# ZechengLi19/CIM

Hardware: AMD Instinct MI355X
Metric: images/sec training step (ResNet-50 VOC, ~1k proposals/img) at 1/2/4/8 GPU (higher is better)
Workload: dtype fp32

## Files before the change

### cim_amd/_lib.py

```python
import ctypes
import os

from ctypes import c_float, c_int, c_longlong, c_void_p

HERE = os.path.dirname(os.path.abspath(__file__))
LIB_PATH = os.environ.get("CIM_HIP_LIB") or os.path.join(HERE, "libcim_hip.so")

_P = c_void_p
SIGNATURES = {
    "cim_roi_align_fwd": [_P, _P, _P] + [c_int] * 6 + [c_float, c_int, c_int, _P],
    "cim_roi_align_fwd_ws": [_P, _P, _P] + [c_int] * 6 + [c_float, c_int, c_int, _P, _P],
    "cim_roi_align_maskcat_fwd_ws": [_P, _P, _P, _P] + [c_int] * 6 + [c_float, c_int, c_int, _P, _P],
    "cim_roi_align_wino7_pair_fwd": [_P, _P, _P, _P, _P] + [c_int] * 7 + [c_float, c_int, c_int, _P, _P],
    "cim_roi_align_bwd_ws": [_P, _P, _P] + [c_int] * 6 + [c_float, c_int, c_int, _P, c_int, _P, _P],
    "cim_roi_align_maskcat_bwd_ws": [_P, _P, _P, _P] + [c_int] * 6 + [c_float, c_int, c_int, _P, c_int, _P, _P],
    "cim_roi_align_bwd_workspace": [c_int, c_int, c_int, c_int],
    "cim_roi_align_bwd_scratch": [c_int, c_int, c_int, c_int, c_int],
    "cim_roi_align_bwd": [_P, _P, _P] + [c_int] * 6 + [c_float, c_int, c_int, _P, _P],
    "cim_roi_align_maskcat_fwd": [_P, _P, _P, _P] + [c_int] * 6 + [c_float, c_int, c_int, _P],
    "cim_roi_align_maskcat_bwd": [_P, _P, _P, _P] + [c_int] * 6 + [c_float, c_int, c_int, _P, _P],
    "cim_roi_align_forms": [c_int] * 9 + [_P] * 3,
    "cim_maxpool2d_out_size": [c_int, c_int, c_int, c_int],
    "cim_maxpool2d_fwd": [_P, _P, _P, c_int, c_int, c_int, c_int, c_int, c_int, _P],
    "cim_maxpool2d_bwd": [_P, _P, _P, c_int, c_int, c_int, c_int, c_int, c_int, _P],
    "cim_upsample_nearest_fwd": [_P, _P, c_int, c_int, c_int, c_int, c_int, _P],
    "cim_upsample_nearest_bwd": [_P, _P, c_int, c_int, c_int, c_int, _P],
    "cim_image_prep": [_P, c_int, c_int, _P, c_int, c_int, c_longlong, c_int, ctypes.c_double, c_int, _P, _P],
    "cim_mask_pack": [_P, _P, c_int, c_int, _P],
    "cim_mask_iou_pair": [_P, c_int, c_int, _P, _P, _P, _P],
    "cim_asy_flag": [_P, c_int, c_float, _P, _P],
    "cim_asy_prep": [_P, c_int, _P, c_int, _P, _P, _P],
    "cim_mining_step": [_P, _P, _P],
    "cim_mining_lds_bytes": [c_int, c_int],
    "cim_mining_sync_bytes": [],
    "cim_gemm_small_splits": [c_int, c_int, c_int],
    "cim_gemm_small_f32": [_P, _P, _P] + [c_int] * 8 + [_P, _P, _P, _P, _P, c_float, _P, c_int, c_int, _P, _P],
    "cim_conv1x1_bwd_workspace": [c_int, c_int, c_int, c_int],
    "cim_conv1x1_bn_act_bwd": [_P] * 8 + [c_float, c_int] + [_P] * 5 + [c_int] * 4 + [_P, _P, _P, _P, _P, c_int] + [c_int, _P, _P, c_float] + [_P] * 4 + [c_int],
    "cim_bn_part_finish": [_P, c_int, _P],
    "cim_conv3x3_nchw_splits": [c_int] * 5,
    "cim_conv3x3_nchw_f32": [_P, _P, _P] + [c_int] * 6 + [_P, _P, _P, _P, _P, c_float, _P, c_int, c_int, _P, _P],
    "cim_conv7x7_nchw_f32": [_P, _P, _P] + [c_int] * 5 + [_P, _P, _P, _P, c_float, c_int, _P],
    "cim_conv3x3_nchw_bwd_workspace": [c_int] * 6,
    "cim_conv3x3_dx_parts": [c_int] * 3,
    "cim_conv3x3_nchw_bn_act_bwd": [_P] * 8 + [c_float, c_int] + [_P] * 5 + [c_int] * 7 + [_P, _P, _P, _P, _P, c_int] + [c_int, _P, _P, c_float] + [_P] * 4,
    "cim_conv3x3_wt_multi": [_P, c_int, _P],
    "cim_bn_act_fwd": [_P, _P, _P, _P, _P, _P, c_float, _P, c_int, c_int, c_int, c_int, _P],
    "cim_bn_act_bwd_chunks": [c_int, c_int, c_int],
    "cim_bn_act_bwd": [_P, _P, _P, _P, _P, _P, c_float, _P, _P, _P, _P, c_int, c_int, c_int, c_int, _P],
    "cim_sgd_multi": [_P, _P, c_int, c_float, c_int, _P],
    "cim_adam_multi": [_P, _P, c_int, ctypes.c_double, ctypes.c_double, ctypes.c_double, c_int, _P],
    "cim_gemm_pair_splits": [c_int, c_int, c_int],
    "cim_gemm_pair": [_P, _P, _P, _P] + [c_int] * 6 + [c_int, c_int, c_int, c_int, _P, _P, _P, _P, c_int, c_int, c_int, _P],
    "cim_gemm_pair_batched": [_P, _P, _P] + [c_int] * 6 + [c_int, c_int, c_int, c_longlong, c_longlong, c_longlong,
                              _P, _P, c_int, c_int, c_int, _P],
    "cim_pair_scales": [_P, c_int, _P, _P, c_int, c_int, _P],
    "cim_pair_split": [_P, _P, c_int, c_int, c_int, c_int, c_int, c_int, c_longlong, c_longlong, _P, _P, _P],
    "cim_pair_amax": [_P, c_longlong, _P, _P],
    "cim_pair_masked_stats": [_P, _P, c_int, c_int, _P, _P, _P],
    "cim_wino7_flatten_bwd_dy_pair": [_P, _P, _P, _P, _P, _P, _P, c_int, c_int, c_int, _P],
    "cim_wino7_pair_scales": [_P, c_int, _P, c_int, _P, _P],
    "cim_wino7_input_pair": [_P, _P, _P, c_int, c_int, c_int, _P],
    "cim_wino7_filter_pair": [_P, _P, _P, c_int, c_int, _P],
    "cim_wino7_dy_pair": [_P, _P, _P, c_int, c_int, c_int, c_int, _P],
    "cim_wino7_output_amax": [_P, _P, _P, c_int, c_int, c_int, _P, _P],
    "cim_flatten_chw_pair": [_P, _P, _P, c_int, c_int, c_int, c_int, _P],
    "cim_flatten_chw_bwd_bias": [_P, _P, _P, _P, c_int, c_int, c_int, _P],
    "cim_wino_dx_adjoint_output": [_P, _P, c_int, c_int, c_int, c_int, _P],
    "cim_wino7_dx_maskfold": [_P, _P, _P, c_int, c_int, _P],
    "cim_wino_wgrad_output": [_P, _P, c_int, c_int, c_int, _P],
    "cim_losses_fwd": [_P, _P],
    "cim_linear_bias_f32": [_P, _P, _P, _P, c_int, c_int, c_int, c_int, _P, _P],
    "cim_loss_finish": [_P, c_int, _P, _P],
    "cim_loss_grad_combine": [_P] * 8 + [c_int, c_int, c_int, _P],
    "cim_head_act_fwd": [_P, _P, _P, c_int, c_int, c_int, _P],
    "cim_head_act_bwd": [_P, _P, _P, _P, c_int, c_int, c_int, _P],
    "cim_detect_ws_bytes": [c_int, c_int],
    "cim_detect_nms_limit": [_P, c_int, _P, c_int, c_int, c_float, c_float, c_int, _P, _P, _P, _P, _P],
    "cim_detect_corloc": [_P, c_int, c_int, c_int, _P, _P],
    "cim_batch_detect_ws_bytes": [_P, c_int, c_int],
    "cim_batch_detect_nms_limit": [_P, c_int, _P, _P, _P, c_int, c_int, c_float, c_float, c_int, _P, _P, _P, _P, _P, _P, _P],
    "cim_segm_words": [c_int, c_int],
    "cim_segm_pack": [_P, _P, c_longlong, c_int, c_int, c_int, _P, _P],
    "cim_segm_area": [_P, c_int, c_int, _P, _P],
    "cim_segm_rle_count": [_P, c_int, c_int, c_int, _P, _P],
    "cim_segm_rle_write": [_P, c_int, c_int, c_int, _P, _P, _P, _P],
    "cim_segm_rle_decode_ws_bytes": [c_longlong],
    "cim_segm_rle_decode": [_P, _P, _P, c_int, c_int, c_int, _P, _P, _P],
    "cim_segm_image_ws_bytes": [c_int, c_int, c_longlong],
    "cim_segm_record_bytes": [c_int, c_int, c_int, c_int],
    "cim_segm_eval_image": [_P, c_int, _P, c_int, c_int, _P, _P, c_int, c_int, c_int, c_longlong, _P, _P, _P, c_int, _P, c_int,
                            _P, _P, _P],
    "cim_segm_accumulate_ws_bytes": [c_longlong, c_int, c_int, c_int],
    "cim_segm_accumulate": [_P, c_int, c_longlong, c_int, _P, _P, _P, c_int, _P, c_int, _P, c_int, c_int, c_int, _P, _P, _P, _P,
                            _P],
    "cim_poly_ws_bytes": [c_int, c_int, c_int],
    "cim_poly_fill": [_P, _P, _P, _P, c_int, c_int, c_longlong, c_int, c_int, c_int, _P, _P, _P],
    "cim_box_image_ws_bytes": [c_int, c_int, c_longlong],
    "cim_box_eval_image": [_P, c_int, _P, c_int, _P, _P, c_int, c_int, c_int, c_longlong, _P, _P, _P, c_int, _P, c_int, _P, _P, _P],
    "cim_voc_match": [_P, _P, c_int, _P, _P, c_int, _P, c_int, ctypes.c_double, c_int, _P, _P, _P, _P, _P],
    "cim_voc_ap_ws_bytes": [c_longlong],
    "cim_voc_ap": [_P, _P, _P, c_longlong, _P, _P, c_int, _P, c_int, _P, _P, c_int, _P, _P, _P, _P, _P, _P],
    "cim_prop_ws_bytes": [c_int, c_int, c_int],
    "cim_prop_prepare": [_P, c_int, c_int, c_int, c_int, _P, _P, _P, _P, _P, _P, _P],
    "cim_prop_assign": [_P, _P, c_int, c_int, c_int, _P, _P, _P, c_int, c_int, _P, _P, _P],
}

ABI_VERSION = 16
_lib = None


class CimHipError(RuntimeError):
    pass


def load():
    global _lib
    if _lib is not None:
        return _lib
    import torch
    if not os.path.exists(LIB_PATH):
        raise CimHipError(
            "libcim_hip.so not found at %s - build it with `python -m cim_amd.build` "
            "(there is no CPU fallback for the CIM hot path)" % LIB_PATH)
    lib = ctypes.CDLL(LIB_PATH)
    lib.cim_last_error.restype = ctypes.c_char_p
    lib.cim_last_error.argtypes = []
    lib.cim_abi_version.restype = c_int
    if lib.cim_abi_version() != ABI_VERSION:
        raise CimHipError("%s exports ABI %d, this package binds ABI %d: rebuild with `python -m cim_amd.build`"
                          % (LIB_PATH, lib.cim_abi_version(), ABI_VERSION))
    for name, argtypes in SIGNATURES.items():
        fn = getattr(lib, name)
        fn.argtypes = argtypes
        fn.restype = c_longlong if name in ("cim_conv1x1_bwd_workspace", "cim_conv3x3_nchw_bwd_workspace", "cim_roi_align_bwd_workspace", "cim_roi_align_bwd_scratch", "cim_mining_lds_bytes", "cim_mining_sync_bytes", "cim_detect_ws_bytes") or name in _LONG_RETURNING else c_int
    _lib = lib
    return lib


_LONG_RETURNING = {"cim_segm_rle_decode_ws_bytes", "cim_segm_image_ws_bytes", "cim_segm_record_bytes", "cim_segm_accumulate_ws_bytes", "cim_prop_ws_bytes", "cim_poly_ws_bytes", "cim_box_image_ws_bytes",
                   "cim_voc_ap_ws_bytes", "cim_batch_detect_ws_bytes"}
VALUE_RETURNING = _LONG_RETURNING | {"cim_segm_words"} | {"cim_maxpool2d_out_size", "cim_conv3x3_dx_parts", "cim_mining_sync_bytes", "cim_conv1x1_bwd_workspace", "cim_conv3x3_nchw_bwd_workspace", "cim_conv3x3_nchw_splits", "cim_gemm_small_splits", "cim_mining_lds_bytes", "cim_bn_act_bwd_chunks", "cim_gemm_pair_splits", "cim_roi_align_bwd_workspace", "cim_roi_align_bwd_scratch", "cim_detect_ws_bytes"}


PURE = {"cim_maxpool2d_out_size", "cim_conv3x3_dx_parts", "cim_gemm_small_splits", "cim_conv3x3_nchw_splits", "cim_conv1x1_bwd_workspace", "cim_conv3x3_nchw_bwd_workspace",
        "cim_bn_act_bwd_chunks", "cim_gemm_pair_splits"}
_PURE_VALUES = {}


def call(name, *args):
    if name in PURE:
        key = (name,) + args
        v = _PURE_VALUES.get(key)
# ... 22 lines not shown
```

### cim_amd/csrc/winograd.hip

```cpp
#include "common.h"
#include "../../include/cim_hip.h"
#include "wino7_tile.h"

namespace {

__device__ __forceinline__ float4 f4(float v) { return make_float4(v, v, v, v); }
__device__ __forceinline__ void fma2(float2& a, float s, float2 v) { a.x = fmaf(s, v.x, a.x); a.y = fmaf(s, v.y, a.y); }

typedef float w7_v2 __attribute__((ext_vector_type(2)));
typedef float w7_v4 __attribute__((ext_vector_type(4)));

constexpr int W7_VOUT = 4;
constexpr int W7_VDX = 2;
constexpr int W7_VMF = 1;
constexpr int W7_MF_WAVES = 1;
constexpr int W7_FB_WAVES = 3;
constexpr int W7_WG_CI = 4;

template <int N> struct w7_vec;
template <> struct w7_vec<1> { typedef float T; };
template <> struct w7_vec<2> { typedef float2 T; };
template <> struct w7_vec<4> { typedef float4 T; };
__device__ __forceinline__ void w7_store(float* p, float v) { __builtin_nontemporal_store(v, p); }
__device__ __forceinline__ void w7_store(float* p, float2 v) { __builtin_nontemporal_store(w7_v2{v.x, v.y}, reinterpret_cast<w7_v2*>(p)); }
// ... 286 lines not shown
__device__ __forceinline__ void w7_dx_tile(const float* __restrict__ M, size_t MC, size_t rc, VT (&acc)[7][7]) {
    constexpr int NA = W7::NP[KA], NB = W7::NP[KB], P = 7, Q0 = W7::QOFF[KA * 2 + KB];
    VT q[NA][NB];
#pragma unroll
    for (int i = 0; i < NA; ++i)
#pragma unroll
        for (int j = 0; j < NB; ++j) q[i][j] = vload_once<VT>(M + (size_t)(Q0 + i * NB + j) * MC + rc);
#pragma unroll
    for (int k = 0; k < NA; ++k) {
        const int yy = W7::IN0[KA] + k;
        if (yy < 0 || yy >= P) continue;
        VT t[NB];
#pragma unroll
        for (int j = 0; j < NB; ++j) {
            vzero(t[j]);
#pragma unroll
            for (int i = 0; i < NA; ++i)
                if (W7_BT[KA][i][k] != 0.0f) vfma(t[j], W7_BT[KA][i][k], q[i][j]);
        }
#pragma unroll
        for (int l = 0; l < NB; ++l) {
            const int xx = W7::IN0[KB] + l;
            if (xx < 0 || xx >= P) continue;
#pragma unroll
            for (int j = 0; j < NB; ++j)
                if (W7_BT[KB][j][l] != 0.0f) vfma(acc[yy][xx], W7_BT[KB][j][l], t[j]);
        }
    }
}

__global__ __launch_bounds__(256) void wino7_dx_kernel(const float* __restrict__ M, float* __restrict__ dx, int R, int C) {
    constexpr int VW = W7_VDX;
    typedef typename w7_vec<VW>::T VT;
    const int r = blockIdx.x;
    const size_t MC = (size_t)R * C;
    for (int c = (blockIdx.y * 256 + threadIdx.x) * VW; c < C; c += gridDim.y * 256 * VW) {
        VT acc[7][7];
#pragma unroll
        for (int y = 0; y < 7; ++y)
#pragma unroll
            for (int x = 0; x < 7; ++x) vzero(acc[y][x]);
        const size_t rc = (size_t)r * C + c;
        w7_for_all_tiles([&](auto t) __attribute__((always_inline)) { w7_dx_tile<t.KA, t.KB, VT>(M, MC, rc, acc); });
#pragma unroll
        for (int y = 0; y < 7; ++y)
#pragma unroll
            for (int x = 0; x < 7; ++x) w7_store(dx + (((size_t)r * 7 + y) * 7 + x) * C + c, acc[y][x]);
    }
}

__global__ __launch_bounds__(256, W7_MF_WAVES) void wino7_dx_maskfold_kernel(const float* __restrict__ M, const float* __restrict__ masks,
                                                                float* __restrict__ dbox, int R, int Cb) {
    constexpr int VW = W7_VMF;
    typedef typename w7_vec<VW>::T VT;
    const int r = blockIdx.x;
    const size_t C2 = 2 * (size_t)Cb, MC = (size_t)R * C2;
    const float* __restrict__ mk = masks + (size_t)r * 49;
    for (int c = (blockIdx.y * 256 + threadIdx.x) * VW; c < Cb; c += gridDim.y * 256 * VW) {
        VT acc[7][7];
#pragma unroll
        for (int y = 0; y < 7; ++y)
#pragma unroll
            for (int x = 0; x < 7; ++x) vzero(acc[y][x]);
        const size_t rc = (size_t)r * C2 + c;
        w7_for_all_tiles([&](auto t) __attribute__((always_inline)) { w7_dx_tile<t.KA, t.KB, VT>(M, MC, rc + Cb, acc); });
#pragma unroll
        for (int y = 0; y < 7; ++y)
#pragma unroll
            for (int x = 0; x < 7; ++x) {
                const float m = mk[y * 7 + x];
                VT z;
                vzero(z);
                vfma(z, m, acc[y][x]);
                acc[y][x] = z;
            }
        w7_for_all_tiles([&](auto t) __attribute__((always_inline)) { w7_dx_tile<t.KA, t.KB, VT>(M, MC, rc, acc); });
#pragma unroll
        for (int y = 0; y < 7; ++y)
#pragma unroll
            for (int x = 0; x < 7; ++x) w7_store(dbox + (((size_t)r * 7 + y) * 7 + x) * Cb + c, acc[y][x]);
    }
}

template <int KA, int KB, typename VT>
__device__ __forceinline__ void w7_wgrad_tile(const float* __restrict__ dU, size_t KN, size_t idx, VT (&acc)[3][3]) {
    constexpr int NA = W7::NP[KA], NB = W7::NP[KB], Q0 = W7::QOFF[KA * 2 + KB];
    VT s[3][NB];
#pragma unroll
    for (int a = 0; a < 3; ++a)
#pragma unroll
        for (int j = 0; j < NB; ++j) vzero(s[a][j]);
#pragma unroll
    for (int i = 0; i < NA; ++i)
#pragma unroll
        for (int j = 0; j < NB; ++j) {
            const VT q = vload_once<VT>(dU + (size_t)(Q0 + i * NB + j) * KN + idx);
#pragma unroll
            for (int a = 0; a < 3; ++a)
                if (W7_AW[KA][a][i] != 0.0f) vfma(s[a][j], W7_AW[KA][a][i], q);
        }
#pragma unroll
    for (int a = 0; a < 3; ++a)
#pragma unroll
        for (int b = 0; b < 3; ++b)
#pragma unroll
            for (int j = 0; j < NB; ++j)
                if (W7_AW[KB][b][j] != 0.0f) vfma(acc[a][b], W7_AW[KB][b][j], s[a][j]);
}

__global__ __launch_bounds__(256) void wino7_wgrad_out_kernel(const float* __restrict__ dU, float* __restrict__ dW, int Cout,
                                                              int Cin) {
    const size_t idx = (size_t)blockIdx.x * 256 + threadIdx.x;
    const size_t KN = (size_t)Cin * Cout;
    if (idx >= KN) return;
    const int ci = (int)(idx / Cout), co = (int)(idx % Cout);
    float acc[3][3];
#pragma unroll
    for (int a = 0; a < 3; ++a)
#pragma unroll
        for (int b = 0; b < 3; ++b) acc[a][b] = 0.0f;
    w7_for_all_tiles([&](auto t) __attribute__((always_inline)) { w7_wgrad_tile<t.KA, t.KB, float>(dU, KN, idx, acc); });
    float* dst = dW + ((size_t)co * Cin + ci) * 9;
#pragma unroll
    for (int a = 0; a < 3; ++a)
#pragma unroll
        for (int b = 0; b < 3; ++b) dst[a * 3 + b] = acc[a][b];
}

__global__ __launch_bounds__(64 * W7_WG_CI) void wino7_wgrad_out_rows_kernel(const float* __restrict__ dU, float* __restrict__ dW,
                                                                                 int Cout, int Cin) {
    constexpr int NCI = W7_WG_CI, ROW = 9 * NCI;
    __shared__ float t[64][ROW + 1];
    const int lane = threadIdx.x & 63, w = threadIdx.x >> 6;
    const int co0 = blockIdx.x * 64, ci0 = blockIdx.y * NCI;
    const size_t KN = (size_t)Cin * Cout;
    const size_t idx = (size_t)(ci0 + w) * Cout + co0 + lane;
    float acc[3][3];
#pragma unroll
    for (int a = 0; a < 3; ++a)
#pragma unroll
        for (int b = 0; b < 3; ++b) acc[a][b] = 0.0f;
    w7_for_all_tiles([&](auto t) __attribute__((always_inline)) { w7_wgrad_tile<t.KA, t.KB, float>(dU, KN, idx, acc); });
#pragma unroll
    for (int a = 0; a < 3; ++a)
#pragma unroll
        for (int b = 0; b < 3; ++b) t[lane][w * 9 + a * 3 + b] = acc[a][b];
    __syncthreads();
    for (int e = threadIdx.x; e < 64 * ROW; e += 64 * NCI) {
        const int row = e / ROW, col = e - row * ROW;
        dW[((size_t)(co0 + row) * Cin + ci0) * 9 + col] = t[row][col];
    }
}

__global__ __launch_bounds__(256) void flatten_chw_bwd_kernel(const float* __restrict__ src, const float* __restrict__ y,
                                                              float* __restrict__ dst, int PP, int C, float* __restrict__ bsum) {
    __shared__ float t[64][65];
    const int r = blockIdx.x, c0 = blockIdx.y * 64, tid = threadIdx.x;
    const size_t base = (size_t)r * PP * C;
    for (int e = tid; e < PP * 64; e += 256) {
        const int c = e / PP, p = e - c * PP;
        t[p][c] = src[base + (size_t)c0 * PP + e];
    }
    __syncthreads();
    float part = 0.0f;
    for (int e = tid; e < PP * 64; e += 256) {
        const int p = e >> 6, c = e & 63;
        const size_t o = base + (size_t)p * C + c0 + c;
        const float v = (y == nullptr || y[o] > 0.0f) ? t[p][c] : 0.0f;
        dst[o] = v;
        part += v;
    }
    if (bsum != nullptr) {
        __syncthreads();
        t[tid >> 6][tid & 63] = part;
        __syncthreads();
        if (tid < 64) bsum[(size_t)r * C + c0 + tid] = (t[0][tid] + t[1][tid]) + (t[2][tid] + t[3][tid]);
    }
}

__global__ __launch_bounds__(256) void flatten_chw_pair_kernel(const float* __restrict__ src, float* __restrict__ dst, int R,
                                                               int PP, int C, const float* __restrict__ scale) {
    __shared__ float t[64][65];
    const int r = blockIdx.x, c0 = blockIdx.y * 64, tid = threadIdx.x;
    float* out = dst + (size_t)r * PP * C + (size_t)c0 * PP;
    const int chunks = PP * 8;
    if (r >= R) {
        for (int q = tid; q < chunks * 2; q += 256) *reinterpret_cast<float4*>(out + q * 4) = make_float4(0.f, 0.f, 0.f, 0.f);
        return;
    }
    const size_t base = (size_t)r * PP * C;
    for (int e = tid; e < PP * 64; e += 256) {
        const int p = e >> 6, c = e & 63;
        t[p][c] = src[base + (size_t)p * C + c0 + c];
    }
    __syncthreads();
    const float s = scale[0];
    for (int q = tid; q < chunks; q += 256) {
        float v[8];
#pragma unroll
        for (int k = 0; k < 8; ++k) {
            const int e = q * 8 + k, c = e / PP, p = e - c * PP;
            v[k] = t[p][c] * s;
        }
        unsigned hh[4], ll[4];
#pragma unroll
        for (int e = 0; e < 4; ++e) cim::pair_split2(v[2 * e], v[2 * e + 1], hh[e], ll[e]);
        const w7_u4 h = {hh[0], hh[1], hh[2], hh[3]}, l = {ll[0], ll[1], ll[2], ll[3]};
        *reinterpret_cast<w7_u4*>(out + q * 8) = h;
        *reinterpret_cast<w7_u4*>(out + q * 8 + 4) = l;
    }
}

}

extern "C" int cim_wino_wgrad_output(const float* dU, float* dW, int Cout, int Cin, int tile, void* stream) {
    CIM_CHECK_ARG(dU && dW && Cout > 0 && Cin > 0);
    CIM_CHECK_ARG(tile == 7);
    const size_t n = (size_t)Cout * Cin;
    if (Cout % 64 == 0 && Cin % W7_WG_CI == 0 && Cin / W7_WG_CI <= 65535)
        hipLaunchKernelGGL(wino7_wgrad_out_rows_kernel, dim3(Cout / 64, Cin / W7_WG_CI), dim3(64 * W7_WG_CI), 0, cim::as_stream(stream), dU,
                           dW, Cout, Cin);
    else hipLaunchKernelGGL(wino7_wgrad_out_kernel, dim3((unsigned)((n + 255) / 256)), dim3(256), 0, cim::as_stream(stream), dU, dW, Cout, Cin);
    CIM_CHECK_LAUNCH();
    return 0;
}

extern "C" int cim_wino_dx_adjoint_output(const float* M, float* dx, int R, int P, int C, int tile, void* stream) {
    CIM_CHECK_ARG(R > 0 && P > 0 && P <= 64 && C > 0 && C % 4 == 0);
    CIM_CHECK_ARG(M && dx && tile == 7 && P == 7 && R <= 2147483647);
    int chunks = (C + 256 * W7_VDX - 1) / (256 * W7_VDX);
    if (chunks > 4) chunks = 4;
    hipLaunchKernelGGL(wino7_dx_kernel, dim3(R, chunks), dim3(256), 0, cim::as_stream(stream), M, dx, R, C);
    CIM_CHECK_LAUNCH();
    return 0;
}

extern "C" int cim_wino7_dx_maskfold(const float* M, const float* masks, float* dbox, int R, int Cb, void* stream) {
    CIM_CHECK_ARG(M && masks && dbox && R > 0 && Cb > 0 && Cb % 4 == 0);
    int chunks = (Cb + 256 * W7_VMF - 1) / (256 * W7_VMF);
    if (chunks > 4) chunks = 4;
    hipLaunchKernelGGL(wino7_dx_maskfold_kernel, dim3(R, chunks), dim3(256), 0, cim::as_stream(stream), M, masks, dbox, R, Cb);
    CIM_CHECK_LAUNCH();
    return 0;
}

extern "C" int cim_wino7_pair_scales(const uint32_t* amax, int n_amax, const uint32_t* amax_mul, int kind, float* scale, void* stream) {
    CIM_CHECK_ARG(amax && scale && kind >= 0 && kind <= 3 && n_amax >= 1 && n_amax <= 65536);
    hipLaunchKernelGGL(wino7_pair_scales_kernel, dim3(1), dim3(128), 0, cim::as_stream(stream), amax, n_amax, amax_mul, kind, scale);
    CIM_CHECK_LAUNCH();
    return 0;
}

extern "C" int cim_wino7_input_pair(const float* x, void* V, const float* scale, int R, int Rs, int C, void* stream) {
    CIM_CHECK_ARG(x && V && scale && R > 0 && Rs >= R && C > 0 && C % 8 == 0);
    hipLaunchKernelGGL(wino7_input_pair_kernel, dim3(Rs, 4), dim3(256), 0, cim::as_stream(stream), x, (float*)V, R, Rs, C, scale);
    CIM_CHECK_LAUNCH();
    return 0;
}

extern "C" int cim_wino7_filter_pair(const float* W, void* U, const float* scale, int Cout, int Cin, void* stream) {
    CIM_CHECK_ARG(W && U && scale && Cout > 0 && Cin > 0 && Cin % 8 == 0);
    const size_t n = (size_t)Cout * Cin;
    hipLaunchKernelGGL(wino7_filter_pair_kernel, dim3((unsigned)((n + 255) / 256)), dim3(256), 0, cim::as_stream(stream), W,
                       (float*)U, Cout, Cin, scale);
    CIM_CHECK_LAUNCH();
    return 0;
}

extern "C" int cim_wino7_dy_pair(const float* dy, void* D, const float* scale, int R, int Rs, int C, int adjoint, void* stream) {
    CIM_CHECK_ARG(dy && D && scale && R > 0 && Rs >= R && C > 0 && C % 8 == 0);
    if (adjoint) hipLaunchKernelGGL(wino7_dy_pair_kernel<true>, dim3(Rs, 4), dim3(256), 0, cim::as_stream(stream), dy, (float*)D, R, Rs, C, scale);
    else hipLaunchKernelGGL(wino7_dy_pair_kernel<false>, dim3(Rs, 4), dim3(256), 0, cim::as_stream(stream), dy, (float*)D, R, Rs, C, scale);
    CIM_CHECK_LAUNCH();
    return 0;
}

extern "C" int cim_wino7_flatten_bwd_dy_pair(const float* dX, const float* relu_y, void* E, const float* scale_e, void* D,
                                             const float* scale_d, float* bias_partial, int R, int Rs, int C, void* stream) {
    CIM_CHECK_ARG(dX && (E || D) && (!E || scale_e) && (!D || scale_d) && R > 0 && Rs >= R && C > 0 && C % 256 == 0 && C / 256 <= 65535);
    hipLaunchKernelGGL(wino7_flatten_bwd_dy_pair_kernel, dim3(Rs, C / 256), dim3(256), 0, cim::as_stream(stream), dX, relu_y, (float*)E,
                       (float*)D, bias_partial, R, Rs, C, scale_e, scale_d);
    CIM_CHECK_LAUNCH();
    return 0;
}

extern "C" int cim_wino7_output_amax(const float* M, const float* bias, float* y, int R, int C, int relu, uint32_t* y_amax,
                                     void* stream) {
    CIM_CHECK_ARG(M && y && R > 0 && C > 0 && C % 4 == 0);
    hipLaunchKernelGGL(wino7_output_kernel, dim3(R, 4), dim3(256), 0, cim::as_stream(stream), M, bias, y, R, C, relu, y_amax);
    CIM_CHECK_LAUNCH();
    return 0;
}

extern "C" int cim_flatten_chw_pair(const float* src, void* dst, const float* scale, int R, int Rs, int PP, int C, void* stream) {
    CIM_CHECK_ARG(src && dst && scale && R > 0 && Rs >= R && PP > 0 && PP <= 64 && C > 0 && C % 64 == 0 && C / 64 <= 65535);
    hipLaunchKernelGGL(flatten_chw_pair_kernel, dim3(Rs, C / 64), dim3(256), 0, cim::as_stream(stream), src, (float*)dst, R, PP, C, scale);
    CIM_CHECK_LAUNCH();
    return 0;
}

extern "C" int cim_flatten_chw_bwd_bias(const float* src, const float* relu_y, float* dst, float* bias_partial, int R, int PP,
                                        int C, void* stream) {
    CIM_CHECK_ARG(src && dst && R > 0 && PP > 0 && PP <= 64 && C > 0 && C % 64 == 0 && C / 64 <= 65535);
    hipLaunchKernelGGL(flatten_chw_bwd_kernel, dim3(R, C / 64), dim3(256), 0, cim::as_stream(stream), src, relu_y, dst, PP, C, bias_partial);
    CIM_CHECK_LAUNCH();
    return 0;
}
// ... 1 lines not shown
```

### cim_amd/ops/maskfuse_pair.py

```python
import torch
from torch.autograd import Function

from .. import _lib
from . import chain
from . import gemm as G
from . import pair

NPOS = 121
DEFER_DW = True
DW_WGS = 256
DW_FORM = 1
DW_FORM1_WGS = 0
import collections as _collections
SCHEDULE = _collections.Counter()


def supported(cat, wc, w1, w2):
    r, cin, p, q = cat.shape
    cout = wc.shape[0]
    return (cat.is_cuda and p == 7 and q == 7 and cin % 32 == 0 and cout % 64 == 0 and wc.shape[1] == cin
            and w1.shape[1] == cout * 49 and w1.shape[0] % 32 == 0 and w2.shape[1] == w1.shape[0] and w2.shape[0] % 32 == 0)


def _weight_amax(w, rows, cols):
# ... 170 lines not shown
            G.run_postponed(gcat.device)
        return dfeat, None, None, dwc, dbc, dw1, db1, dw2, db2, None, None, None


def _head_backward(ctx, dY2, ofs, fold_masks=None):
    if True:
        (y, Y1, Y2, Vb, Vs, Ub, Us, W1b, W1s, W2b, W2s, Xb, Xs, Y1b, Y1s) = ctx.saved_tensors
        r, cin, cout, h1, h2, p = ctx.dims
        dev, rp = y.device, pair.pad32(r)
        V = pair.Pair(Vb, r, cin, NPOS, Vs)
        Up = pair.Pair(Ub, cout, cin, NPOS, Us)
        W1p, W2p = pair.Pair(W1b, h1, cout * p * p, 1, W1s), pair.Pair(W2b, h2, h1, 1, W2s)
        Xp, Y1p = pair.Pair(Xb, r, cout * p * p, 1, Xs), pair.Pair(Y1b, r, h1, 1, Y1s)
        need_x, need_wc, need_w1, need_w2 = ctx.needs_input_grad[0], ctx.needs_input_grad[1 + ofs], ctx.needs_input_grad[3 + ofs], ctx.needs_input_grad[5 + ofs]
        cur, side = torch.cuda.current_stream(dev), G._side_stream(dev)
        overlap = G.OVERLAP and not torch.cuda.is_current_stream_capturing()

        def on_side(fn):
            if not overlap:
                return fn()
            side.wait_stream(cur)
            with torch.cuda.stream(side):
                out = fn()
            return out

        def publish(w, dw):
            pub = publisher
            if pub is None or dw is None or not isinstance(w, torch.nn.Parameter) or not w.is_leaf:
                return dw
            if pub(w, dw, side if overlap else cur):
                published.append(dw)
                SCHEDULE["weight_gradients_published_early"] += 1
                return None
            return dw

        published = []
        publisher = G.publisher_for(ctx.weights[1])
        if publisher is not None and chain.restricted_pass(ctx, (1 + ofs, 3 + ofs, 5 + ofs)):
            publisher = None
        late = []
        restricted = chain.restricted_pass(ctx, (1 + ofs, 3 + ofs, 5 + ofs))
        defer = DEFER_DW and G.DEFER_DW and not restricted
        run_late = overlap and defer and DW_WGS > 0

        def side_grad(slot, w, fn):
            if run_late:
                late.append((slot, w, fn))
                return None
            return publish(w, on_side(fn))

        wc_p, w1_p, w2_p = ctx.weights
        dcat = dwc = dbc = dw1 = db1 = dw2 = db2 = None
        needed = [w for w, need in ((w2_p, need_w2), (w1_p, need_w1), (wc_p, need_wc)) if need]
        will_postpone = (run_late and G.POSTPONE_DW and publisher is None and len(needed) > 0
                         and all(isinstance(w, torch.nn.Parameter) for w in needed))
        bc_p, b1_p, b2_p = getattr(ctx, "biases", (None, None, None))
        late_bias = []

        def bias_sum(b_p, part):
            if part is None:
                return None
            if will_postpone and isinstance(b_p, torch.nn.Parameter):
                late_bias.append((b_p, part, torch.empty(part.shape[1], dtype=part.dtype, device=part.device)))
                return None
            return part.sum(dim=0)
        dy_keep = []
        am = torch.zeros(3, dtype=torch.int32, device=dev)
        dY2 = dY2.contiguous()
        db2 = bias_sum(b2_p, pair.masked_stats(dY2, Y2, am[0:1], ctx.has_bias[2] and ctx.needs_input_grad[6 + ofs], reduce=False))
        dY2p = pair.split(dY2, r, h2, h2, scale=pair.scales_from(am[0:1], 1), relu_y=Y2)
        if need_w2:
            dw2 = side_grad(2, w2_p, lambda limit=0, form=0: pair.gemm(dY2p, Y1p, h2, h1, rp, True, False, limit=limit, form=form))
        dY1 = pair.gemm(dY2p, W2p, r, h1, h2, False, False)
        db1 = bias_sum(b1_p, pair.masked_stats(dY1, Y1, am[1:2], ctx.has_bias[1] and ctx.needs_input_grad[4 + ofs], reduce=False))
        dY1p = pair.split(dY1, r, h1, h1, scale=pair.scales_from(am[1:2], 1), relu_y=Y1)
        if need_w1:
            dw1 = side_grad(1, w1_p, lambda limit=0, form=0: pair.gemm(dY1p, Xp, h1, cout * p * p, rp, True, False, limit=limit, form=form))
        if need_x or need_wc or (ctx.has_bias[0] and ctx.needs_input_grad[2 + ofs]):
            dX = pair.gemm(dY1p, W1p, r, cout * p * p, h1, False, False, c_amax=am[2:3], balance=True)
            st = _lib.stream_ptr()
            want_dbc = ctx.has_bias[0] and ctx.needs_input_grad[2 + ofs]
            bpart = torch.empty((r, cout), dtype=torch.float32, device=dev) if want_dbc else None
            fused = FUSE_DY and cout % 256 == 0 and p == 7
            E = D = dy = None
            if fused:
                if need_x:
                    sE = torch.empty(NPOS, dtype=torch.float32, device=dev)
                    _lib.call("cim_wino7_pair_scales", am[2:3].data_ptr(), 1, None, 3, sE.data_ptr(), st)
                    E = pair.Pair(torch.empty((NPOS, rp, cout), dtype=torch.int32, device=dev), r, cout, NPOS, sE)
                if need_wc:
                    sD = torch.empty(NPOS, dtype=torch.float32, device=dev)
                    _lib.call("cim_wino7_pair_scales", am[2:3].data_ptr(), 1, None, 2, sD.data_ptr(), st)
                    D = pair.Pair(torch.empty((NPOS, rp, cout), dtype=torch.int32, device=dev), r, cout, NPOS, sD)
                if E is not None or D is not None:
                    _lib.call("cim_wino7_flatten_bwd_dy_pair", dX.data_ptr(), y.data_ptr(), _lib.ptr(E.buf if E is not None else None),
                              _lib.ptr(E.scale if E is not None else None), _lib.ptr(D.buf if D is not None else None),
                              _lib.ptr(D.scale if D is not None else None),
                              _lib.ptr(bpart), r, rp, cout, st)
                else:
                    fused = False
            if not fused:
                dy = torch.empty((r, p, p, cout), dtype=torch.float32, device=dev)
                _lib.call("cim_flatten_chw_bwd_bias", dX.data_ptr(), y.data_ptr(), dy.data_ptr(), _lib.ptr(bpart), r, p * p, cout, st)
            del dX
            if want_dbc:
                dbc = bias_sum(bc_p, bpart)
            if need_wc:
                def wgrad(limit=0, form=0, D=D):
                    st2 = _lib.stream_ptr()
                    if D is None:
                        sD = torch.empty(NPOS, dtype=torch.float32, device=dev)
                        _lib.call("cim_wino7_pair_scales", am[2:3].data_ptr(), 1, None, 2, sD.data_ptr(), st2)
                        D = pair.Pair(torch.empty((NPOS, rp, cout), dtype=torch.int32, device=dev), r, cout, NPOS, sD)
                        _lib.call("cim_wino7_dy_pair", dy.data_ptr(), D.buf.data_ptr(), sD.data_ptr(), r, rp, cout, 0, st2)
                    dU = pair.gemm(V, D, cin, cout, rp, True, False, limit=limit, form=form)
                    dw = torch.empty((cout, cin, 3, 3), dtype=torch.float32, device=dev)
                    _lib.call("cim_wino_wgrad_output", dU.data_ptr(), dw.data_ptr(), cout, cin, 7, st2)
                    return dw
                dwc = side_grad(0, wc_p, wgrad)
            if need_x:
                if E is None:
                    sE = torch.empty(NPOS, dtype=torch.float32, device=dev)
                    _lib.call("cim_wino7_pair_scales", am[2:3].data_ptr(), 1, None, 3, sE.data_ptr(), st)
                    E = pair.Pair(torch.empty((NPOS, rp, cout), dtype=torch.int32, device=dev), r, cout, NPOS, sE)
                    _lib.call("cim_wino7_dy_pair", dy.data_ptr(), E.buf.data_ptr(), sE.data_ptr(), r, rp, cout, 1, st)
                M2 = pair.gemm(E, Up, r, cin, cout, False, False, balance=True)
                if fold_masks is None:
                    dxp = torch.empty((r, p, p, cin), dtype=torch.float32, device=dev)
                    _lib.call("cim_wino_dx_adjoint_output", M2.data_ptr(), dxp.data_ptr(), r, p, cin, 7, st)
                else:
                    dxp = torch.empty((r, p, p, cin // 2), dtype=torch.float32, device=dev)
                    _lib.call("cim_wino7_dx_maskfold", M2.data_ptr(), fold_masks.data_ptr(), dxp.data_ptr(), r, cin // 2, st)
                dcat = dxp.permute(0, 3, 1, 2)
            dy_keep = [t for t in ((dy,) if D is None else (D.buf, D.scale)) if t is not None]
            if overlap:
                for t in dy_keep:
                    t.record_stream(side)
        keep_alive = [t for t in (V.buf, V.scale, Xp.buf, Xp.scale, Y1p.buf, Y1p.scale, dY2p.buf, dY2p.scale, dY1p.buf, dY1p.scale, am)
                      if t is not None] + dy_keep
        if late:
            late.sort(key=lambda e: -e[1].numel())

            def launch(defer):
                c2 = torch.cuda.current_stream(dev)
                late_st = G._late_stream(dev) if publisher is None else side
                late_st.wait_stream(c2)
                if late_st is not side:
                    late_st.wait_stream(side)
                    for t in keep_alive:
                        t.record_stream(late_st)
                with torch.cuda.stream(late_st):
                    limit = (G.LATE_CUS or DW_WGS) if publisher is None else 0
                    form = DW_FORM
                    if form == 1:
                        limit = DW_FORM1_WGS
                    SCHEDULE["late_launches_chunked" if publisher is None else "late_launches_whole_products"] += 1
                    got = {slot: publish(w, fn(limit, form)) for slot, w, fn in late}
                    if defer:
                        for b_p, part, out in late_bias:
                            part.record_stream(late_st)
                            out.record_stream(late_st)
                            torch.sum(part, dim=0, out=out)
                if defer:
                    for b_p, part, out in late_bias:
                        G.defer_side_join(dev, b_p, out, part)
                    keep = [t for t in (V.buf, V.scale, Xp.buf, Xp.scale, Y1p.buf, Y1p.scale, dY2p.buf, dY2p.scale, dY1p.buf,
                                        dY1p.scale, am) if t is not None] + dy_keep
                    for slot, w, _ in late:
                        if got[slot] is not None:
                            G.defer_side_join(dev, w, got[slot], *keep)
                return got

            if G.POSTPONE_DW and publisher is None and all(isinstance(w, torch.nn.Parameter) for _, w, _ in late):
                SCHEDULE["late_launches_postponed_behind_roi_align"] += 1
                G.postpone(dev, lambda: launch(True))
            else:
                assert not late_bias, "bias partial sums were left to a postponed launch that does not happen"
                got = launch(False)
                dwc, dw1, dw2 = got.get(0, dwc), got.get(1, dw1), got.get(2, dw2)
        else:
            assert not late_bias, "bias partial sums were left to a postponed launch that does not happen"
        if overlap:
            for t in [V.buf, V.scale, Xp.buf, Xp.scale, Y1p.buf, Y1p.scale, dY2p.buf, dY2p.scale, dY1p.buf, dY1p.scale, am] + dy_keep:
                if t is not None:
                    t.record_stream(side)
            if defer:
                keep = [V.buf, Xp.buf, Y1p.buf, dY2p.buf, dY1p.buf] + dy_keep
                for w, t in ((w2_p, dw2), (w1_p, dw1), (wc_p, dwc)):
                    if t is not None and isinstance(w, torch.nn.Parameter):
                        G.defer_side_join(dev, w, t, *[k for k in keep if k is not None])
                dw2 = None if isinstance(w2_p, torch.nn.Parameter) else dw2
                dw1 = None if isinstance(w1_p, torch.nn.Parameter) else dw1
                dwc = None if isinstance(wc_p, torch.nn.Parameter) else dwc
                if any(t is not None for t in (dw2, dw1, dwc)):
                    cur.wait_stream(side)
            else:
                cur.wait_stream(side)
                for t in (dw2, dw1, dwc):
                    if t is not None:
                        t.record_stream(cur)
        return dcat, dwc, dbc, dw1, db1, dw2, db2


def maskfuse_head(cat, conv, fc1, fc2, feat_amax):
    return MaskFusePairFunction.apply(cat, conv.weight, conv.bias, fc1.weight, fc1.bias, fc2.weight, fc2.bias, feat_amax)


def roi_supported(x, conv_w, fc1_w, fc2_w, resolution):
    c, h, w = x.shape[1], x.shape[2], x.shape[3]
    cout = conv_w.shape[0]
    return (x.is_cuda and x.dtype == torch.float32 and resolution == 7 and c % 32 == 0 and h <= 128 and w <= 128 and h * w * c < (1 << 30)
            and cout % 64 == 0 and conv_w.shape[1] == 2 * c and fc1_w.shape[1] == cout * 49 and fc1_w.shape[0] % 32 == 0
            and fc2_w.shape[1] == fc1_w.shape[0] and fc2_w.shape[0] % 32 == 0)


def maskfuse_roi_head(x, rois, masks, conv, fc1, fc2, feat_amax, spatial_scale, sampling_ratio):
    return MaskFuseRoiPairFunction.apply(x, rois, masks, conv.weight, conv.bias, fc1.weight, fc1.bias, fc2.weight, fc2.bias,
# ... 2 lines not shown
```

### include/cim_hip.h

```cpp
#ifndef CIM_HIP_H
#define CIM_HIP_H

#include <stdint.h>

#ifdef __cplusplus
extern "C" {
#endif

const char* cim_last_error(void);
int cim_abi_version(void);

int cim_roi_align_fwd(const float* feat, const float* rois, float* out,
                      int B, int C, int H, int W, int K, int P,
                      float spatial_scale, int sampling_ratio, int aligned, void* stream);

long long cim_roi_align_bwd_workspace(int K, int P, int H, int W);
int cim_roi_align_bwd(const float* grad_out, const float* rois, float* grad_in,
                      int B, int C, int H, int W, int K, int P,
                      float spatial_scale, int sampling_ratio, int aligned, float* workspace, void* stream);

int cim_roi_align_fwd_ws(const float* feat, const float* rois, float* out,
                         int B, int C, int H, int W, int K, int P,
                         float spatial_scale, int sampling_ratio, int aligned, float* workspace, void* stream);
int cim_roi_align_maskcat_fwd_ws(const float* feat, const float* rois, const float* masks, float* cat,
// ... 139 lines not shown
int cim_prop_prepare(const uint8_t* masks_u8, int N, int H, int W, int S, uint64_t* packed, int32_t* boxes, int32_t* area,
                     uint8_t* small, int32_t* empty_flag, void* ws, void* stream);
int cim_prop_assign(const uint64_t* packed, const int32_t* area, int N, int H, int W, const int32_t* rows, const int32_t* cols,
                    const int32_t* classes, int P, int C, float* mat, void* ws, void* stream);

int cim_image_prep(const uint8_t* src_bgr, int h, int w, float* dst, int H, int W, long long plane_stride, int row_stride,
                   double inv_scale, int hflip, const float* mean_std6_host, void* stream);

int cim_maxpool2d_out_size(int in, int k, int stride, int pad);
int cim_maxpool2d_fwd(const float* x, float* y, int* idx, int NC, int H, int W, int k, int stride, int pad, void* stream);
int cim_maxpool2d_bwd(const float* dy, const int* idx, float* dx, int NC, int H, int W, int k, int stride, int pad, void* stream);
int cim_upsample_nearest_fwd(const float* x, float* y, int NC, int H, int W, int scale, int accumulate, void* stream);
int cim_upsample_nearest_bwd(const float* dy, float* dx, int NC, int H, int W, int scale, void* stream);

int cim_gemm_small_splits(int M, int N, int K);
int cim_gemm_small_f32(const float* A, const float* B, float* C, int M, int N, int K, int lda, int ldb, int ldc,
                       int a_mcontig, int b_kcontig, float* x_raw, const float* gamma, const float* beta,
                       const float* mean, const float* var, float eps, const float* residual, int relu, int splits,
                       float* workspace, void* stream);

long long cim_conv1x1_bwd_workspace(int B, int cin, int cout, int hw);
int cim_conv1x1_bn_act_bwd(const float* dy, const float* y, const float* x_raw, const float* x, const float* w,
                           const float* gamma, const float* mean, const float* var, float eps, int relu,
                           float* dres, float* dgamma, float* dbeta, float* dx, float* dw, int B, int cin, int cout, int hw,
                           float* workspace, void* stream, void* side_stream, void* fork_event, void* join_event, int join,
                           int dy_is_dconv, const float* in_gamma, const float* in_var, float in_eps,
                           const float* in_xr, const float* in_mean, float* in_part, const float* dx_add, int dx_add_w);
typedef struct { const float* part; const float* var; float eps; float* dgamma; float* dbeta; int images; int parts; int channels; } cim_bn_part_desc;
int cim_bn_part_finish(const cim_bn_part_desc* descs, int n, void* stream);

int cim_conv3x3_nchw_splits(int cin, int cout, int H, int W, int stride);
int cim_conv3x3_nchw_f32(const float* x, const float* w, float* y, int cin, int cout, int H, int W, int stride, int dilation,
                         float* x_raw, const float* gamma, const float* beta, const float* mean, const float* var, float eps,
                         const float* residual, int relu, int splits, float* workspace, void* stream);
int cim_conv7x7_nchw_f32(const float* x, const float* w, float* y, int cin, int cout, int H, int W, int stride,
                         const float* gamma, const float* beta, const float* mean, const float* var, float eps, int relu,
                         void* stream);
long long cim_conv3x3_nchw_bwd_workspace(int B, int cin, int cout, int H, int W, int stride);
int cim_conv3x3_dx_parts(int H, int W, int stride);
int cim_conv3x3_nchw_bn_act_bwd(const float* dy, const float* y, const float* x_raw, const float* x, const float* w,
                                const float* gamma, const float* mean, const float* var, float eps, int relu, float* dres,
                                float* dgamma, float* dbeta, float* dx, float* dw, int B, int cin, int cout, int H, int W,
                                int stride, int dilation, float* workspace, void* stream, void* side_stream, void* fork_event,
                                void* join_event, int join, int dy_is_dconv, const float* in_gamma, const float* in_var, float in_eps,
                                const float* in_xr, const float* in_mean, float* in_part, const float* wt_ready);
typedef struct { const float* w; float* wt; int cin; int cout; } cim_wt_desc;
int cim_conv3x3_wt_multi(const cim_wt_desc* descs, int n, void* stream);

int cim_bn_act_fwd(const float* x, const float* res, const float* gamma, const float* beta, const float* mean,
                   const float* var, float eps, float* y, int N, int C, int HW, int relu, void* stream);
int cim_bn_act_bwd_chunks(int N, int C, int HW);
int cim_bn_act_bwd(const float* dy, const float* y, const float* x, const float* gamma, const float* mean,
                   const float* var, float eps, float* dx, float* dres, float* dgamma, float* dbeta,
                   int N, int C, int HW, int relu, void* stream);

int cim_gemm_pair_splits(int M, int N, int K);
int cim_gemm_pair(const void* A, const void* B, float* C, const float* bias, int M, int N, int K,
                  int lda, int ldb, int ldc, int a_mcontig, int b_kcontig, int relu, int splits, float* workspace,
                  const float* a_scale, const float* b_scale, uint32_t* c_amax, int max_workgroups, int products, int form,
                  void* stream);
int cim_gemm_pair_batched(const void* A, const void* B, float* C, int M, int N, int K,
                          int lda, int ldb, int ldc, int a_mcontig, int b_kcontig,
                          int batch, long long a_bs, long long b_bs, long long c_bs,
                          const float* a_scale, const float* b_scale, int max_workgroups, int products, int form, void* stream);
int cim_pair_scales(const uint32_t* amax, int n_amax, const float* factor, float* scale, int n, int reduce_all, void* stream);
int cim_pair_split(const float* X, void* P, int rows, int rows_pad, int cols, int ld, int ldp, int batch,
                   long long x_bs, long long p_bs, const float* scale, const float* relu_y, void* stream);
int cim_pair_amax(const float* X, long long n, uint32_t* amax, void* stream);
int cim_pair_masked_stats(const float* dy, const float* y, int rows, int cols, float* part, uint32_t* amax, void* stream);

int cim_wino7_pair_scales(const uint32_t* amax, int n_amax, const uint32_t* amax_mul, int kind, float* scale, void* stream);
int cim_wino7_input_pair(const float* x, void* V, const float* scale, int R, int Rs, int C, void* stream);
int cim_wino7_filter_pair(const float* W, void* U, const float* scale, int Cout, int Cin, void* stream);
int cim_wino7_dy_pair(const float* dy, void* D, const float* scale, int R, int Rs, int C, int adjoint, void* stream);
int cim_wino7_flatten_bwd_dy_pair(const float* dX, const float* relu_y, void* E, const float* scale_e, void* D, const float* scale_d,
                                  float* bias_partial, int R, int Rs, int C, void* stream);
int cim_wino7_output_amax(const float* M, const float* bias, float* y, int R, int C, int relu, uint32_t* y_amax, void* stream);
int cim_flatten_chw_pair(const float* src, void* dst, const float* scale, int R, int Rs, int PP, int C, void* stream);
int cim_flatten_chw_bwd_bias(const float* src, const float* relu_y, float* dst, float* bias_partial, int R, int PP, int C,
                             void* stream);


int cim_wino_wgrad_output(const float* dU, float* dW, int Cout, int Cin, int tile, void* stream);
int cim_wino_dx_adjoint_output(const float* M, float* dx, int R, int P, int C, int tile, void* stream);
int cim_wino7_dx_maskfold(const float* M, const float* masks, float* dbox, int R, int Cb, void* stream);

#define CIM_PCL_MAX_CLUSTERS 256
typedef struct cim_loss_args {
    const float* pc;
    const float* pd;
    const float* rc[3];
    const float* ri[3];
    const float* pseudo_labels[3];
    const uint16_t* pseudo_iou_f16[3];
    const float* loss_weights[3];
    float weight_scale[3];
    const int32_t* layer_valid;
    const float* labels;
    const float* mat;
    int32_t* status;
    int N, C1, R;
    float* part;
    float* grad;
    int ld;
} cim_loss_args;

int cim_losses_fwd(const cim_loss_args* args, void* stream);

int cim_linear_bias_f32(const float* X, const float* W, const float* bias, float* Y, int M, int N, int K, int splits,
                        float* workspace, void* stream);
int cim_loss_finish(const float* part, int rows, float* out, void* stream);
int cim_loss_grad_combine(const float* G, const float* g_bag, const float* g_pcl, const float* g_cls, const float* g_iou,
                          const float* g_iou3, const float* g_total, float* out, int N, int C1, int R, void* stream);
int cim_head_act_fwd(const float* logits, float* scores, float* colstat, int N, int C1, int R, void* stream);
int cim_head_act_bwd(const float* scores, const float* grad_scores, float* grad_logits, float* coldot,
                     int N, int C1, int R, void* stream);

typedef struct cim_sgd_tensor {
    uint64_t p;
    uint64_t g;
    uint64_t buf;
    int64_t n;
    float lr, wd;
    int32_t rows, cols;
    uint64_t row_amax, col_amax;
} cim_sgd_tensor;
typedef struct cim_sgd_chunk {
    int32_t tensor;
    int32_t n;
    int64_t offset;
} cim_sgd_chunk;
int cim_sgd_multi(const cim_sgd_tensor* tensors, const cim_sgd_chunk* chunks, int n_chunks, float momentum, int max_workgroups,
                  void* stream);

typedef struct cim_adam_tensor {
    uint64_t p;
    uint64_t g;
    uint64_t exp_avg;
    uint64_t exp_avg_sq;
    int64_t n;
    float step_size, bc2_sqrt, wd;
    int32_t rows, cols;
    int32_t reserved;
    uint64_t row_amax, col_amax;
} cim_adam_tensor;
int cim_adam_multi(const cim_adam_tensor* tensors, const cim_sgd_chunk* chunks, int n_chunks, double beta1, double beta2, double eps,
                   int max_workgroups, void* stream);

#ifdef __cplusplus
}
#endif
#endif
```

Measured before the change: 76.06.

## Reuse adjoint-transformed dy pair for both weight and input gradients

The backward pass of the fused mask conv used to build two Winograd-transformed copies of dy, one with the forward transform (D) for the weight gradient and one with the adjoint transform (E) for the input gradient. It now builds only E and computes the weight gradient from it. A new templated wgrad output kernel applies the transposed G matrix instead of the AW matrix to undo the adjoint transform. This removes one transform pass, one quantized buffer, and its scale computation. The cost is possible numeric differences from quantizing with the adjoint scale, and the side stream now depends on the E buffer.

New measurement: 76.81 (median of 6 runs). Within noise of the previous version (+1.0%).

```diff
diff --git a/cim_amd/_lib.py b/cim_amd/_lib.py
--- a/cim_amd/_lib.py
+++ b/cim_amd/_lib.py
@@ -69,6 +69,7 @@
     "cim_wino_dx_adjoint_output": [_P, _P, c_int, c_int, c_int, c_int, _P],
     "cim_wino7_dx_maskfold": [_P, _P, _P, c_int, c_int, _P],
     "cim_wino_wgrad_output": [_P, _P, c_int, c_int, c_int, _P],
+    "cim_wino_wgrad_output_adj": [_P, _P, c_int, c_int, c_int, _P],
     "cim_losses_fwd": [_P, _P],
     "cim_linear_bias_f32": [_P, _P, _P, _P, c_int, c_int, c_int, c_int, _P, _P],
     "cim_loss_finish": [_P, c_int, _P, _P],
diff --git a/cim_amd/csrc/winograd.hip b/cim_amd/csrc/winograd.hip
--- a/cim_amd/csrc/winograd.hip
+++ b/cim_amd/csrc/winograd.hip
@@ -392,7 +392,7 @@
     }
 }
 
-template <int KA, int KB, typename VT>
+template <int KA, int KB, bool ADJ, typename VT>
 __device__ __forceinline__ void w7_wgrad_tile(const float* __restrict__ dU, size_t KN, size_t idx, VT (&acc)[3][3]) {
     constexpr int NA = W7::NP[KA], NB = W7::NP[KB], Q0 = W7::QOFF[KA * 2 + KB];
     VT s[3][NB];
@@ -406,18 +406,23 @@
         for (int j = 0; j < NB; ++j) {
             const VT q = vload_once<VT>(dU + (size_t)(Q0 + i * NB + j) * KN + idx);
 #pragma unroll
-            for (int a = 0; a < 3; ++a)
-                if (W7_AW[KA][a][i] != 0.0f) vfma(s[a][j], W7_AW[KA][a][i], q);
+            for (int a = 0; a < 3; ++a) {
+                const float m = ADJ ? W7_G[KA][i][a] : W7_AW[KA][a][i];
+                if (m != 0.0f) vfma(s[a][j], m, q);
+            }
         }
 #pragma unroll
     for (int a = 0; a < 3; ++a)
 #pragma unroll
         for (int b = 0; b < 3; ++b)
 #pragma unroll
-            for (int j = 0; j < NB; ++j)
-                if (W7_AW[KB][b][j] != 0.0f) vfma(acc[a][b], W7_AW[KB][b][j], s[a][j]);
-}
-
+            for (int j = 0; j < NB; ++j) {
+                const float m = ADJ ? W7_G[KB][j][b] : W7_AW[KB][b][j];
+                if (m != 0.0f) vfma(acc[a][b], m, s[a][j]);
+            }
+}
+
+template <bool ADJ>
 __global__ __launch_bounds__(256) void wino7_wgrad_out_kernel(const float* __restrict__ dU, float* __restrict__ dW, int Cout,
                                                               int Cin) {
     const size_t idx = (size_t)blockIdx.x * 256 + threadIdx.x;
@@ -429,7 +434,7 @@
     for (int a = 0; a < 3; ++a)
 #pragma unroll
         for (int b = 0; b < 3; ++b) acc[a][b] = 0.0f;
-    w7_for_all_tiles([&](auto t) __attribute__((always_inline)) { w7_wgrad_tile<t.KA, t.KB, float>(dU, KN, idx, acc); });
+    w7_for_all_tiles([&](auto t) __attribute__((always_inline)) { w7_wgrad_tile<t.KA, t.KB, ADJ, float>(dU, KN, idx, acc); });
     float* dst = dW + ((size_t)co * Cin + ci) * 9;
 #pragma unroll
     for (int a = 0; a < 3; ++a)
@@ -437,6 +442,7 @@
         for (int b = 0; b < 3; ++b) dst[a * 3 + b] = acc[a][b];
 }
 
+template <bool ADJ>
 __global__ __launch_bounds__(64 * W7_WG_CI) void wino7_wgrad_out_rows_kernel(const float* __restrict__ dU, float* __restrict__ dW,
                                                                                  int Cout, int Cin) {
     constexpr int NCI = W7_WG_CI, ROW = 9 * NCI;
@@ -450,7 +456,7 @@
     for (int a = 0; a < 3; ++a)
 #pragma unroll
         for (int b = 0; b < 3; ++b) acc[a][b] = 0.0f;
-    w7_for_all_tiles([&](auto t) __attribute__((always_inline)) { w7_wgrad_tile<t.KA, t.KB, float>(dU, KN, idx, acc); });
+    w7_for_all_tiles([&](auto t) __attribute__((always_inline)) { w7_wgrad_tile<t.KA, t.KB, ADJ, float>(dU, KN, idx, acc); });
 #pragma unroll
     for (int a = 0; a < 3; ++a)
 #pragma unroll
@@ -521,18 +527,27 @@
     }
 }
 
-}
-
-extern "C" int cim_wino_wgrad_output(const float* dU, float* dW, int Cout, int Cin, int tile, void* stream) {
+template <bool ADJ>
+int w7_launch_wgrad_output(const float* dU, float* dW, int Cout, int Cin, int tile, void* stream) {
     CIM_CHECK_ARG(dU && dW && Cout > 0 && Cin > 0);
     CIM_CHECK_ARG(tile == 7);
     const size_t n = (size_t)Cout * Cin;
     if (Cout % 64 == 0 && Cin % W7_WG_CI == 0 && Cin / W7_WG_CI <= 65535)
-        hipLaunchKernelGGL(wino7_wgrad_out_rows_kernel, dim3(Cout / 64, Cin / W7_WG_CI), dim3(64 * W7_WG_CI), 0, cim::as_stream(stream), dU,
+        hipLaunchKernelGGL(wino7_wgrad_out_rows_kernel<ADJ>, dim3(Cout / 64, Cin / W7_WG_CI), dim3(64 * W7_WG_CI), 0, cim::as_stream(stream), dU,
                            dW, Cout, Cin);
-    else hipLaunchKernelGGL(wino7_wgrad_out_kernel, dim3((unsigned)((n + 255) / 256)), dim3(256), 0, cim::as_stream(stream), dU, dW, Cout, Cin);
-    CIM_CHECK_LAUNCH();
-    return 0;
+    else hipLaunchKernelGGL(wino7_wgrad_out_kernel<ADJ>, dim3((unsigned)((n + 255) / 256)), dim3(256), 0, cim::as_stream(stream), dU, dW, Cout, Cin);
+    CIM_CHECK_LAUNCH();
+    return 0;
+}
+
+}
+
+extern "C" int cim_wino_wgrad_output(const float* dU, float* dW, int Cout, int Cin, int tile, void* stream) {
+    return w7_launch_wgrad_output<false>(dU, dW, Cout, Cin, tile, stream);
+}
+
+extern "C" int cim_wino_wgrad_output_adj(const float* dU, float* dW, int Cout, int Cin, int tile, void* stream) {
+    return w7_launch_wgrad_output<true>(dU, dW, Cout, Cin, tile, stream);
 }
 
 extern "C" int cim_wino_dx_adjoint_output(const float* M, float* dx, int R, int P, int C, int tile, void* stream) {
diff --git a/cim_amd/ops/maskfuse_pair.py b/cim_amd/ops/maskfuse_pair.py
--- a/cim_amd/ops/maskfuse_pair.py
+++ b/cim_amd/ops/maskfuse_pair.py
@@ -276,48 +276,31 @@
             want_dbc = ctx.has_bias[0] and ctx.needs_input_grad[2 + ofs]
             bpart = torch.empty((r, cout), dtype=torch.float32, device=dev) if want_dbc else None
             fused = FUSE_DY and cout % 256 == 0 and p == 7
-            E = D = dy = None
-            if fused:
-                if need_x:
-                    sE = torch.empty(NPOS, dtype=torch.float32, device=dev)
-                    _lib.call("cim_wino7_pair_scales", am[2:3].data_ptr(), 1, None, 3, sE.data_ptr(), st)
-                    E = pair.Pair(torch.empty((NPOS, rp, cout), dtype=torch.int32, device=dev), r, cout, NPOS, sE)
-                if need_wc:
-                    sD = torch.empty(NPOS, dtype=torch.float32, device=dev)
-                    _lib.call("cim_wino7_pair_scales", am[2:3].data_ptr(), 1, None, 2, sD.data_ptr(), st)
-                    D = pair.Pair(torch.empty((NPOS, rp, cout), dtype=torch.int32, device=dev), r, cout, NPOS, sD)
-                if E is not None or D is not None:
-                    _lib.call("cim_wino7_flatten_bwd_dy_pair", dX.data_ptr(), y.data_ptr(), _lib.ptr(E.buf if E is not None else None),
-                              _lib.ptr(E.scale if E is not None else None), _lib.ptr(D.buf if D is not None else None),
-                              _lib.ptr(D.scale if D is not None else None),
-                              _lib.ptr(bpart), r, rp, cout, st)
-                else:
-                    fused = False
-            if not fused:
+            E = None
+            if need_x or need_wc:
+                sE = torch.empty(NPOS, dtype=torch.float32, device=dev)
+                _lib.call("cim_wino7_pair_scales", am[2:3].data_ptr(), 1, None, 3, sE.data_ptr(), st)
+                E = pair.Pair(torch.empty((NPOS, rp, cout), dtype=torch.int32, device=dev), r, cout, NPOS, sE)
+            if fused and E is not None:
+                _lib.call("cim_wino7_flatten_bwd_dy_pair", dX.data_ptr(), y.data_ptr(), E.buf.data_ptr(), E.scale.data_ptr(), None, None,
+                          _lib.ptr(bpart), r, rp, cout, st)
+            else:
                 dy = torch.empty((r, p, p, cout), dtype=torch.float32, device=dev)
                 _lib.call("cim_flatten_chw_bwd_bias", dX.data_ptr(), y.data_ptr(), dy.data_ptr(), _lib.ptr(bpart), r, p * p, cout, st)
+                if E is not None:
+                    _lib.call("cim_wino7_dy_pair", dy.data_ptr(), E.buf.data_ptr(), E.scale.data_ptr(), r, rp, cout, 1, st)
+                del dy
             del dX
             if want_dbc:
                 dbc = bias_sum(bc_p, bpart)
             if need_wc:
-                def wgrad(limit=0, form=0, D=D):
-                    st2 = _lib.stream_ptr()
-                    if D is None:
-                        sD = torch.empty(NPOS, dtype=torch.float32, device=dev)
-                        _lib.call("cim_wino7_pair_scales", am[2:3].data_ptr(), 1, None, 2, sD.data_ptr(), st2)
-                        D = pair.Pair(torch.empty((NPOS, rp, cout), dtype=torch.int32, device=dev), r, cout, NPOS, sD)
-                        _lib.call("cim_wino7_dy_pair", dy.data_ptr(), D.buf.data_ptr(), sD.data_ptr(), r, rp, cout, 0, st2)
-                    dU = pair.gemm(V, D, cin, cout, rp, True, False, limit=limit, form=form)
+                def wgrad(limit=0, form=0):
+                    dU = pair.gemm(V, E, cin, cout, rp, True, False, limit=limit, form=form)
                     dw = torch.empty((cout, cin, 3, 3), dtype=torch.float32, device=dev)
-                    _lib.call("cim_wino_wgrad_output", dU.data_ptr(), dw.data_ptr(), cout, cin, 7, st2)
+                    _lib.call("cim_wino_wgrad_output_adj", dU.data_ptr(), dw.data_ptr(), cout, cin, 7, _lib.stream_ptr())
                     return dw
                 dwc = side_grad(0, wc_p, wgrad)
             if need_x:
-                if E is None:
-                    sE = torch.empty(NPOS, dtype=torch.float32, device=dev)
-                    _lib.call("cim_wino7_pair_scales", am[2:3].data_ptr(), 1, None, 3, sE.data_ptr(), st)
-                    E = pair.Pair(torch.empty((NPOS, rp, cout), dtype=torch.int32, device=dev), r, cout, NPOS, sE)
-                    _lib.call("cim_wino7_dy_pair", dy.data_ptr(), E.buf.data_ptr(), sE.data_ptr(), r, rp, cout, 1, st)
                 M2 = pair.gemm(E, Up, r, cin, cout, False, False, balance=True)
                 if fold_masks is None:
                     dxp = torch.empty((r, p, p, cin), dtype=torch.float32, device=dev)
@@ -326,7 +309,7 @@
                     dxp = torch.empty((r, p, p, cin // 2), dtype=torch.float32, device=dev)
                     _lib.call("cim_wino7_dx_maskfold", M2.data_ptr(), fold_masks.data_ptr(), dxp.data_ptr(), r, cin // 2, st)
                 dcat = dxp.permute(0, 3, 1, 2)
-            dy_keep = [t for t in ((dy,) if D is None else (D.buf, D.scale)) if t is not None]
+            dy_keep = [E.buf, E.scale] if need_wc else []
             if overlap:
                 for t in dy_keep:
                     t.record_stream(side)
diff --git a/include/cim_hip.h b/include/cim_hip.h
--- a/include/cim_hip.h
+++ b/include/cim_hip.h
@@ -245,6 +245,7 @@
 
 
 int cim_wino_wgrad_output(const float* dU, float* dW, int Cout, int Cin, int tile, void* stream);
+int cim_wino_wgrad_output_adj(const float* dU, float* dW, int Cout, int Cin, int tile, void* stream);
 int cim_wino_dx_adjoint_output(const float* M, float* dx, int R, int P, int C, int tile, void* stream);
 int cim_wino7_dx_maskfold(const float* M, const float* masks, float* dbox, int R, int Cb, void* stream);
 
```
